# kiliant/zklaim

Hardware: AMD Instinct MI355X
Metric: Groth16 proofs/sec (zklaim gadget, alt_bn128) + G1 MSM GB/s vs HBM roofline (higher is better)
Workload: dtype u32 limbs, Montgomery (254-bit Fq/Fr: 9 x 29-bit in the accumulation, reduction and NTT kernels, 8 x 32-bit elsewhere)

## Files before the change

### zklaim_amd/csrc/msm.hip

```cpp
#include "common.hpp"
#include "fq29.hip.hpp"
#include "host/horner_jac.hpp"
#include "../../include/zkg.h"
#include <algorithm>
#include <chrono>
#include <cstdio>
#include <cstdlib>
#include <cstring>
#include <mutex>

#define ZK_VGPR_CAP(n) __attribute__((amdgpu_num_vgpr((n) / 2)))
static constexpr int ACC29_VGPRS = 192;

namespace zk {

static constexpr int SCALAR_BITS = 255;
template <class F> struct RedGeom { static constexpr int LANES_LOG = sizeof(F) == sizeof(Fq) ? 7 : 6, LANES = 1 << LANES_LOG, THREADS = 4 * LANES; };
static constexpr int RED_L_LOG_TINY = 0, RED_L_LOG_SMALL = 2, RED_L_LOG_LARGE = 4;
static constexpr size_t RED_SMALL_BUCKETS = (size_t)1 << 16, RED_LARGE_BUCKETS = (size_t)1 << 18;
static constexpr int MAX_C = 16;
static constexpr uint32_t HEAVY_S = 512;
static constexpr uint32_t HEAVY_T_MAX = 1024;
static constexpr uint32_t CLASS_HIST_COPIES = 8;
static constexpr int HEAVY_PART_BLOCKS = 512, HEAVY_MERGE_BLOCKS = 128;
// ... 465 lines not shown
    if (cnt > RX_FINE_MAX) { rx_fine_big_bin(tmp, fbits, start, cnt, gb0, cf, of, cur, counts, offsets, sorted, h, heavy_t, class_hist); return; }
    uint32_t ent[RX_FINE_MAX / T];
#pragma unroll
    for (uint32_t j = 0; j < RX_FINE_MAX / T; ++j) {
        uint32_t p = t + j * T;
        ent[j] = p < cnt ? tmp[start + p] : 0xffffffffu;
        if (p < cnt) atomicAdd(&cf[ent[j] >> sh], 1u);
    }
    __syncthreads();
    rx_fine_offsets(cf, of, FB, t, start, gb0, counts, offsets, h, heavy_t, class_hist);
    __syncthreads();
#pragma unroll
    for (uint32_t j = 0; j < RX_FINE_MAX / T; ++j) {
        if (t + j * T >= cnt) continue;
        uint32_t e = ent[j], f = e >> sh;
        bufB[of[f] + atomicAdd(&cur[f], 1u)] = e & low;
    }
    __syncthreads();
    for (uint32_t p = t; p < cnt; p += T) sorted[start + p] = bufB[p];
}

__global__ __launch_bounds__(1024) void k_class_hist(const uint32_t *counts, const uint32_t *offsets, size_t total, uint32_t *class_hist) {
    sort_wave_priority();
    __shared__ uint32_t h[HEAVY_T_MAX + 2];
    const uint32_t heavy_t = heavy_threshold_dev(offsets, total, 1);
    const uint32_t t = threadIdx.x, nc = heavy_t + 2;
    for (uint32_t i = t; i < nc; i += 1024) h[i] = 0;
    __syncthreads();
    size_t gb = (size_t)blockIdx.x * 1024 + t;
    if (gb < total) { uint32_t c = counts[gb]; atomicAdd(&h[c > heavy_t ? heavy_t + 1 : c], 1u); }
    __syncthreads();
    for (uint32_t i = t; i < nc; i += 1024) if (h[i]) atomicAdd(&class_hist[i], h[i]);
}
__global__ __launch_bounds__(1024) void k_order_place(const uint32_t *counts, const uint32_t *offsets, size_t total, const uint32_t *class_hist, uint32_t *class_cursor,
                                                       uint32_t *order, uint32_t *heavy_out) {
    sort_wave_priority();
    __shared__ uint32_t h[HEAVY_T_MAX + 2], first[HEAVY_T_MAX + 2], wave_total[16], threshold;
    const uint32_t t = threadIdx.x, wave = t >> 6, lane = t & 63;
    for (uint32_t i = t; i < HEAVY_T_MAX + 2; i += 1024) h[i] = 0;
    if (t == 0) threshold = heavy_threshold_dev(offsets, total, 1);
    __syncthreads();
    const uint32_t heavy_t = threshold, nc = heavy_t + 2;
    size_t gb = (size_t)blockIdx.x * 1024 + t;
    uint32_t cls = 0, rank = 0;
    if (gb < total) { uint32_t c = counts[gb]; cls = c > heavy_t ? heavy_t + 1 : c; rank = atomicAdd(&h[cls], 1u); }
    uint32_t v0 = 0, v1 = 0, incl = 0;
    if (128 * wave < nc) {
        for (uint32_t k = 0; k < CLASS_HIST_COPIES; ++k) {
            const uint32_t *copy = class_hist + k * (HEAVY_T_MAX + 2);
            if (2 * t < nc) v0 += copy[nc - 1 - 2 * t];
            if (2 * t + 1 < nc) v1 += copy[nc - 2 - 2 * t];
        }
        if (heavy_out && blockIdx.x == 0 && t == 0) *heavy_out = v0;
        incl = v0 + v1;
        for (uint32_t d = 1; d < 64; d <<= 1) { const uint32_t y = __shfl_up(incl, d, 64); if (lane >= d) incl += y; }
    }
    if (lane == 63) wave_total[wave] = incl;
    __syncthreads();
    if (128 * wave < nc) {
        uint32_t before = incl - v0 - v1;
        for (uint32_t k = 0; k < wave; ++k) before += wave_total[k];
        if (2 * t < nc) first[nc - 1 - 2 * t] = before;
        if (2 * t + 1 < nc) first[nc - 2 - 2 * t] = before + v0;
    }
    __syncthreads();
    for (uint32_t i = t; i < nc; i += 1024) if (h[i]) h[i] = first[i] + atomicAdd(&class_cursor[i], h[i]);
    __syncthreads();
    if (gb < total) order[h[cls] + rank] = (uint32_t)gb;
}

template <class F, bool PLAIN>
__global__ __launch_bounds__(256) void k_bucket_accum(const ViewSet<F> views, const uint32_t *sorted, const uint32_t *offsets, const uint32_t *order,
                                                       size_t lanes , XYZZ<F> *buckets, HeavyItem *items,
                                                       HeavyBucket *heavy, uint32_t *counters , SetLayout L) {
    size_t tid = (size_t)blockIdx.x * blockDim.x + threadIdx.x;
    if (tid >= lanes) return;
    const size_t total_buckets = L.buckets;
    const uint32_t set = blockIdx.y;
    const BaseView<F> bases = views.v[set];
    buckets += set * L.buckets; items += set * L.items; heavy += set * L.heavy; counters += 2 * set;
    const uint32_t heavy_t = heavy_threshold_dev(offsets, total_buckets, sizeof(F) > sizeof(Fq) ? 3 : 1);
    const uint32_t gb = order[tid];
    uint32_t k = offsets[gb], end = offsets[gb + 1];
    if (end - k > heavy_t) {
        uint32_t nparts = (end - k + HEAVY_S - 1) / HEAVY_S;
        uint32_t first = atomicAdd(&counters[0], nparts);
        for (uint32_t p = 0; p < nparts; ++p) { uint32_t a = k + p * HEAVY_S; items[first + p] = {a, a + HEAVY_S < end ? a + HEAVY_S : end, gb, nparts == 1}; }
        if (nparts > 1) heavy[atomicAdd(&counters[1], 1u)] = {gb, first, nparts};
        return;
    }
    XYZZ<F> acc = XYZZ<F>::inf();
    if (k < end) {
        uint32_t e = sorted[k], e_next = k + 1 < end ? sorted[k + 1] : 0;
        Affine<F> p = bases.template load<PLAIN>(e, gb);
        while (true) {
            Affine<F> cur = p; uint32_t ce = e;
            ++k;
            if (k < end) { e = e_next; p = bases.template load<PLAIN>(e, gb); if (k + 1 < end) e_next = sorted[k + 1]; }
            if (ce & 1u) cur.y = cur.y.neg();
            acc.madd(cur);
            if (k >= end) break;
        }
    }
    buckets[gb] = acc.normalized();
}

__global__ __launch_bounds__(256) void k_bases_to29(const Affine<Fq> *in, size_t n, Rec64 *out) {
    size_t i = (size_t)blockIdx.x * blockDim.x + threadIdx.x;
    if (i >= n) return;
    const Affine<Fq> a = in[i];
    store_rec64(out + i, f29::to29(a.x), f29::to29(a.y), a.is_inf());
}
ZK_D Affine29 load29(const Rec64 *bases, uint32_t e) { return load_rec64(bases + (e >> 1)); }
ZK_D Rec64 load29_raw(const Rec64 *bases, uint32_t e) { return load_rec64_raw(bases + (e >> 1)); }
template <int WAVES, bool OUT29>
__global__ __launch_bounds__(256, WAVES) ZK_VGPR_CAP(ACC29_VGPRS) void k_bucket_accum29(const Rec64 *bases, size_t level_stride, uint32_t B, const uint32_t *sorted, const uint32_t *offsets, const uint32_t *order,
                                                         size_t lanes, void *buckets_, HeavyItem *items, HeavyBucket *heavy, uint32_t *counters, SetLayout L, int flags ) {
    crit_wave_priority(flags & 2);
    const int resume = flags & 1;
    size_t tid = (size_t)blockIdx.x * blockDim.x + threadIdx.x;
    if (tid >= lanes) return;
    const uint32_t heavy_t = heavy_threshold_dev(offsets, L.buckets, 1);
    const uint32_t gb = order[tid];
    if (level_stride) bases += (size_t)(gb / B) * level_stride;
    uint32_t k = offsets[gb], end = offsets[gb + 1];
    if (end - k > heavy_t) {
        uint32_t nparts = (end - k + HEAVY_S - 1) / HEAVY_S;
        uint32_t first = atomicAdd(&counters[0], nparts);
        const bool single = nparts == 1 && !resume;
        for (uint32_t p = 0; p < nparts; ++p) { uint32_t a = k + p * HEAVY_S; items[first + p] = {a, a + HEAVY_S < end ? a + HEAVY_S : end, gb, single}; }
        if (!single) heavy[atomicAdd(&counters[1], 1u)] = {gb, first, nparts};
        return;
    }
    XYZZ29 acc; bool inf = true;
    acc.x = acc.y = acc.zz = acc.zzz = Fq29::zero();
    if constexpr (OUT29) {
        if (resume) {
            if (k >= end) return;
            const Bucket29 old = load_bucket29_raw(reinterpret_cast<const Bucket29 *>(buckets_) + gb);
            uint32_t any = 0;
#pragma unroll
            for (int j = 0; j < 9; ++j) { acc.x.v[j] = old.x[j]; acc.y.v[j] = old.y[j]; acc.zz.v[j] = old.zz[j]; acc.zzz.v[j] = old.zzz[j]; any |= old.zz[j]; }
            inf = any == 0;
        }
    }
    if (k < end) {
        uint32_t e = sorted[k], e_next = k + 1 < end ? sorted[k + 1] : 0;
        Rec64 p = load29_raw(bases, e);
        while (true) {
            const Rec64 curw = p; const uint32_t ce = e;
            ++k;
            if (k < end) { e = e_next; p = load29_raw(bases, e); if (k + 1 < end) e_next = sorted[k + 1]; }
            const Affine29 cur = unpack_rec64(curw);
            if (!cur.inf) {
                Fq29 bx, by;
#pragma unroll
                for (int j = 0; j < 9; ++j) { bx.v[j] = cur.x[j]; by.v[j] = cur.y[j]; }
                if (ce & 1u) by = f29::neg(f29::S2_1, by);
                if (__builtin_expect(!acc.madd(bx, by, inf), 0)) {
                    XYZZ<Fq> a32 = {f29::from29(acc.x), f29::from29(acc.y), f29::from29(acc.zz), f29::from29(acc.zzz)};
                    a32.madd(Affine<Fq>{f29::from29(bx), f29::from29(f29::norm(by))});
                    if (a32.is_inf()) inf = true;
                    else { acc.x = f29::to29(a32.x.normalized()); acc.y = f29::to29(a32.y.normalized()); acc.zz = f29::to29(a32.zz.normalized()); acc.zzz = f29::to29(a32.zzz.normalized()); }
                }
            }
            if (k >= end) break;
        }
    }
    if constexpr (OUT29) store_bucket29(reinterpret_cast<Bucket29 *>(buckets_) + gb, acc, inf);
    else {
        XYZZ<Fq> *buckets = reinterpret_cast<XYZZ<Fq> *>(buckets_);
        if (inf) buckets[gb] = XYZZ<Fq>::inf().normalized();
        else buckets[gb] = XYZZ<Fq>{f29::from29(acc.x), f29::from29(acc.y), f29::from29(acc.zz), f29::from29(acc.zzz)};
    }
}

template <class F> struct alignas(16) LdsPoint {
    XYZZ<F> p; uint32_t pad[4];
    ZK_D LdsPoint &operator=(const XYZZ<F> &v) { p = v; return *this; }
    ZK_D operator const XYZZ<F> &() const { return p; }
    ZK_D XYZZ<F> normalized() const { return p.normalized(); }
// ... 230 lines not shown
    }
    xyzz29_add_pair(run, cur, r);
    Half29 Q = run;
    for (uint32_t d = 1; d < RED_LANES; d <<= 1) {
        lds_store_half29(sh + t, Q, r);
        __syncthreads();
        if (t + d < RED_LANES) xyzz29_add_pair(Q, lds_load_half29(sh + t + d, r), r);
        __syncthreads();
    }
    const Half29 P = Q;
    lds_store_half29(sh + t, t >= 1 ? Q : Half29::inf(), r); lds_store_half29(sh + RED_LANES + t, T0, r);
    __syncthreads();
    for (uint32_t d = RED_LANES / 2; d >= 1; d >>= 1) {
        if (t < d) { Half29 a = lds_load_half29(sh + t, r); xyzz29_add_pair(a, lds_load_half29(sh + t + d, r), r); lds_store_half29(sh + t, a, r); }
        else if (t >= RED_LANES / 2 && t < RED_LANES / 2 + d) {
            const uint32_t u = RED_LANES + (t - RED_LANES / 2);
            Half29 a = lds_load_half29(sh + u, r); xyzz29_add_pair(a, lds_load_half29(sh + u + d, r), r); lds_store_half29(sh + u, a, r);
        }
        __syncthreads();
    }
    if (t == 0) lds_store_half29(sh + 1, P, r);
    __syncthreads();
    if (threadIdx.x == 0) {
        XYZZ<Fq> E = store_point29(sh[0].p);
        for (int i = 0; i < RED_L_LOG; ++i) E = E.dbl();
        E.add(store_point29(sh[RED_LANES].p));
        out[2 * (size_t)blockIdx.x] = store_point29(sh[1].p); out[2 * (size_t)blockIdx.x + 1] = E.normalized();
    }
}

__global__ __launch_bounds__(2 * RedGeom<Fq>::LANES) void k_bucket_reduce29l(const Bucket29 *buckets, uint32_t B, uint32_t chunks_per_window, XYZZ<Fq> *out,
                                                                             size_t in_set_stride, size_t out_set_stride, int critical) {
    crit_wave_priority(critical);
    constexpr int RED_LANES = RedGeom<Fq>::LANES, NT = 2 * RED_LANES, PER = 8, RED_CHUNK = NT * PER;
    static_assert(RED_CHUNK == (RED_LANES << RED_L_LOG_LARGE), "the lane-form reduction keeps the large reduction's chunks");
    extern __shared__ unsigned char red_smem[];
    LdsPoint29 *sh = reinterpret_cast<LdsPoint29 *>(red_smem);
    const uint32_t i = threadIdx.x;
    const uint32_t w = blockIdx.x / chunks_per_window, ch = blockIdx.x % chunks_per_window;
    const Bucket29 *X = buckets + blockIdx.y * in_set_stride + (size_t)w * B;
    out += blockIdx.y * out_set_stride;
    {
        const uint32_t base = ch * RED_CHUNK + i * PER;
        XYZZ29q run = XYZZ29q::inf(), T0 = XYZZ29q::inf();
        XYZZ29q cur = load_bucket29<true>(X, base + PER - 1, B, 0);
        for (int j = PER - 1; j >= 1; --j) {
            const XYZZ29q nxt = load_bucket29<true>(X, base + j - 1, B, 0);
            xyzz29_add_lane(run, cur);
            xyzz29_add_lane(T0, run);
            cur = nxt;
        }
        xyzz29_add_lane(run, cur);
        sh[i].p = run; sh[NT + i].p = T0;
    }
    __syncthreads();
    const uint32_t t = i >> 1, r = i & 1;
    const Half29 R1 = lds_load_half29(sh + 2 * t + 1, r);
    Half29 Q = lds_load_half29(sh + 2 * t, r);
    xyzz29_add_pair(Q, R1, r);
    Half29 Tp = lds_load_half29(sh + NT + 2 * t, r);
    xyzz29_add_pair(Tp, lds_load_half29(sh + NT + 2 * t + 1, r), r);
    __syncthreads();
    for (uint32_t d = 1; d < RED_LANES; d <<= 1) {
        lds_store_half29(sh + t, Q, r);
        __syncthreads();
        if (t + d < RED_LANES) xyzz29_add_pair(Q, lds_load_half29(sh + t + d, r), r);
        __syncthreads();
    }
    const Half29 P = Q;
    lds_store_half29(sh + t, Q, r);
    __syncthreads();
    Half29 V = t + 1 < RED_LANES ? lds_load_half29(sh + t + 1, r) : Half29::inf();
    xyzz29_add_pair(V, R1, r);
    if (t >= 1) xyzz29_add_pair(V, Q, r);
    __syncthreads();
    lds_store_half29(sh + t, V, r); lds_store_half29(sh + RED_LANES + t, Tp, r);
    __syncthreads();
    for (uint32_t d = RED_LANES / 2; d >= 1; d >>= 1) {
        if (t < d) { Half29 a = lds_load_half29(sh + t, r); xyzz29_add_pair(a, lds_load_half29(sh + t + d, r), r); lds_store_half29(sh + t, a, r); }
        else if (t >= RED_LANES / 2 && t < RED_LANES / 2 + d) {
            const uint32_t u = RED_LANES + (t - RED_LANES / 2);
            Half29 a = lds_load_half29(sh + u, r); xyzz29_add_pair(a, lds_load_half29(sh + u + d, r), r); lds_store_half29(sh + u, a, r);
        }
        __syncthreads();
    }
    if (t == 0) lds_store_half29(sh + 1, P, r);
    __syncthreads();
    if (threadIdx.x < 3) out[3 * (size_t)blockIdx.x + threadIdx.x] = store_point29(threadIdx.x == 0 ? sh[1].p : threadIdx.x == 1 ? sh[RED_LANES].p : sh[0].p);
}


__global__ __launch_bounds__(256) void k_bucket_fold29(const Bucket29 *buckets, const uint32_t *counts, uint32_t W, uint32_t B, Bucket29 *out, int critical) {
    crit_wave_priority(critical);
    const uint32_t b = (blockIdx.x * blockDim.x + threadIdx.x) >> 1, r = threadIdx.x & 1;
    if (b >= B) return;
    Half29 acc = Half29::inf();
    uint32_t w = 0;
    while (w < W && !counts[(size_t)w * B + b]) ++w;
    Half29 cur = w < W ? load_half29<true>(buckets + (size_t)w * B, b, B, r) : Half29::inf();
    while (w < W) {
        uint32_t nw = w + 1;
        while (nw < W && !counts[(size_t)nw * B + b]) ++nw;
        const Half29 nxt = nw < W ? load_half29<true>(buckets + (size_t)nw * B, b, B, r) : Half29::inf();
        xyzz29_add_pair(acc, cur, r);
        cur = nxt; w = nw;
    }
    uint32_t *o = reinterpret_cast<uint32_t *>(out + b) + 9 * r;
#pragma unroll
    for (int i = 0; i < 9; ++i) { o[i] = acc.c0.v[i]; o[18 + i] = acc.c1.v[i]; }
}

static constexpr uint32_t FOLD_THREADS = 256;
template <class F>
__global__ __launch_bounds__(FOLD_THREADS) void k_bucket_fold(const XYZZ<F> *buckets, const uint32_t *counts, uint32_t W, uint32_t B, uint32_t fold_b_log, XYZZ<F> *out, SetLayout L) {
    extern __shared__ unsigned char red_smem[];
    LdsPoint<F> *sh = reinterpret_cast<LdsPoint<F> *>(red_smem);
    const uint32_t t = threadIdx.x, FB = 1u << fold_b_log, slots = FOLD_THREADS >> fold_b_log;
    const uint32_t bl = t & (FB - 1), slot = t >> fold_b_log, b = blockIdx.x * FB + bl;
    buckets += blockIdx.y * L.buckets; out += blockIdx.y * L.folded;
    XYZZ<F> acc = XYZZ<F>::inf();
    if (b < B) for (uint32_t w = slot; w < W; w += slots) if (counts[(size_t)w * B + b]) acc.add(buckets[(size_t)w * B + b]);
// ... 117 lines not shown
    extern __shared__ unsigned char red_smem[];
    LdsPoint<F> *sh = reinterpret_cast<LdsPoint<F> *>(red_smem);
    XYZZ<F> *partials = partials_all + (size_t)blockIdx.y * vec_stride + (size_t)blockIdx.x * (count + 1), *out = partials + count;
    XYZZ<F> acc = XYZZ<F>::inf();
    for (uint32_t i = threadIdx.x; i < count; i += 256) acc.add(partials[i]);
    sh[threadIdx.x] = acc;
    __syncthreads();
    lds_tree_reduce<F>(sh, 256, threadIdx.x, 256, [] { __syncthreads(); });
    if (threadIdx.x == 0) out[0] = sh[0].normalized();
}

struct MsmGroup {
    DevBuf buckets, folded, red_out, heavy_items, heavy_buckets, heavy_partials;
    DevBuf bases29;
    void *host_red = nullptr; size_t host_cap = 0; bool g2 = false, table = false; int nsets = 0;
    int out_index[MSM_MAX_SETS] = {0};
    int red_slots = 2; size_t red_stride = 0;
    uint32_t cpw = 0, red_windows = 0; size_t nred = 0; int chunk_log = 0;
    int host_reserve(size_t bytes) {
        if (bytes <= host_cap) return 0;
        if (host_red) (void)hipHostFree(host_red);
        host_red = nullptr; host_cap = 0;
        if (!hip_ok(hipHostMalloc(&host_red, bytes + 4096, hipHostMallocDefault), "hipHostMalloc", __FILE__, __LINE__)) return 1;
        host_cap = bytes + 4096;
        return 0;
    }
    void release() {
        for (DevBuf *b : {&buckets, &folded, &red_out, &heavy_items, &heavy_buckets, &heavy_partials, &bases29}) b->release();
        if (host_red) (void)hipHostFree(host_red);
        host_red = nullptr; host_cap = 0;
    }
};
struct MsmSortSpace {
    DevBuf digits, hist, counts, offsets, scan_sums, class_hist, order, sorted, rx_tmp, rx_meta, heavy_counters[2];
    void release() { for (DevBuf *b : {&digits, &hist, &counts, &offsets, &scan_sums, &class_hist, &order, &sorted, &rx_tmp, &rx_meta, &heavy_counters[0], &heavy_counters[1]}) b->release(); }
};
struct MsmLaunchMode {
    hipStream_t sort_stream = nullptr;
    uint32_t *heavy_out = nullptr;
    int window = 0;
    bool resume = false;
    bool defer_reduce = false;
    bool heavy_pair = true;
    bool beside = false;
    bool timed = false;
    uint32_t *stream_waits = nullptr;
};
struct MsmJob {
    hipStream_t stream = nullptr; bool own_stream = false;
    MsmSortSpace space;
    MsmGroup group[2];
    MsmGeom g{}; size_t n = 0;
    int window_hint = 0;
    uint32_t merge_hint = 1, merge = 1;
    hipStream_t aux = nullptr; hipEvent_t ev_fork = nullptr, ev_join = nullptr; bool converted_aside = false;
    bool one_pass_sort = false;
    bool critical = false;
    uint32_t w0 = 0, ws = 1;
    bool empty = false;
    bool dev_finish = false;
    uint32_t multi = 1; size_t multi_stride = 0;
    std::mutex mu;
    int ensure_side() {
        if (aux) return ZKG_OK;
        if (hipStreamCreateWithFlags(&aux, hipStreamNonBlocking) == hipSuccess && hipEventCreateWithFlags(&ev_fork, hipEventDisableTiming) == hipSuccess &&
            hipEventCreateWithFlags(&ev_join, hipEventDisableTiming) == hipSuccess) return ZKG_OK;
        release_side(); set_error("msm: side stream"); return ZKG_ERROR;
    }
    void release_side() {
        if (aux) { (void)hipStreamSynchronize(aux); (void)hipStreamDestroy(aux); }
        if (ev_fork) (void)hipEventDestroy(ev_fork);
        if (ev_join) (void)hipEventDestroy(ev_join);
        aux = nullptr; ev_fork = ev_join = nullptr;
    }
    void release_device() {
        space.release();
        for (MsmGroup &gr : group) gr.release();
        release_side();
    }
};
struct MsmLaunchSets { MsmBases by_field[2][MSM_MAX_SETS]; MsmGeom g{}; size_t n = 0; bool empty = false; MsmSortSpace *space = nullptr; };

template <class F>
static int launch_accumulate(MsmJob *job, MsmGroup &gr, const MsmLaunchSets &ls, const uint32_t *d_gather, const MsmLaunchMode &mode, bool time_it) {
    const MsmSortSpace &sp = *ls.space; const MsmBases *sets = ls.by_field[gr.g2 ? 1 : 0];
    const MsmGeom g = ls.g; const size_t n = ls.n, total_buckets = (size_t)g.W * g.B; const unsigned ns = (unsigned)gr.nsets;
    const uint32_t P = job->multi, BP = g.B * P, Wp = g.W / P;
    hipStream_t s = job->stream;
    size_t n_entries_max = n * g.W;
    const size_t max_heavy = std::min(total_buckets, n_entries_max / (sizeof(F) != sizeof(Fq) ? 4 : 8)) + 1,
                 max_items = max_heavy + n_entries_max / HEAVY_S + 1;
    typedef RedGeom<F> RG;
    gr.table = sets[0].level_stride != 0;
    gr.red_windows = gr.table ? P : g.W;
    const size_t red_buckets = (size_t)gr.red_windows * g.B;
    static const char *force_l = getenv("ZKG_RED_L_LOG");
    const int red_l_log = force_l ? atoi(force_l) : red_buckets >= RED_LARGE_BUCKETS ? RED_L_LOG_LARGE : red_buckets > RED_SMALL_BUCKETS ? RED_L_LOG_SMALL : RED_L_LOG_TINY;
    gr.chunk_log = RG::LANES_LOG + red_l_log;
    gr.cpw = (g.B + (1u << gr.chunk_log) - 1) >> gr.chunk_log; gr.nred = (size_t)gr.red_windows * gr.cpw;
    gr.red_slots = 2;
    SetLayout L; L.buckets = total_buckets; L.items = max_items; L.heavy = max_heavy; L.partials = max_items; L.folded = BP; L.red_out = gr.nred * 3;
    if (gr.heavy_items.reserve(ns * max_items * sizeof(HeavyItem)) || gr.heavy_buckets.reserve(ns * max_heavy * sizeof(HeavyBucket)) ||
        gr.heavy_partials.reserve(ns * max_items * sizeof(XYZZ<F>)) ||
        gr.buckets.reserve(ns * total_buckets * std::max(sizeof(XYZZ<F>), sizeof(Bucket29))) || (job->dev_finish && gr.red_out.reserve(ns * L.red_out * sizeof(XYZZ<F>))) || ((gr.red_stride = L.red_out), false) ||
        (gr.table && gr.folded.reserve(ns * (size_t)BP * std::max(sizeof(XYZZ<F>), sizeof(Bucket29)))) || (!job->dev_finish && gr.host_reserve(ns * L.red_out * sizeof(XYZZ<F>)))) return ZKG_ERROR;
    XYZZ<F> *buckets = gr.buckets.as<XYZZ<F>>();
    uint32_t *heavy_counters = sp.heavy_counters[gr.g2 ? 1 : 0].as<uint32_t>();
    ViewSet<F> views;
    for (unsigned i = 0; i < (unsigned)MSM_MAX_SETS; ++i) {
        const MsmBases &b = sets[i < ns ? i : 0];
        views.v[i] = BaseView<F>{reinterpret_cast<const Affine<F> *>(b.p), b.level_stride, d_gather, b.index_sub, BP, b.remap};
    }
    const size_t lanes = gr.table ? std::min(total_buckets, n_entries_max) : total_buckets;
    bool plain = !d_gather;
    for (unsigned i = 0; i < ns; ++i) plain = plain && sets[i].level_stride == 0 && sets[i].index_sub == 0 && !sets[i].remap;
    bool use29 = false; const Rec64 *rec29 = nullptr; size_t stride29 = 0;
    if constexpr (sizeof(F) == sizeof(Fq)) {
        if (ns == 1 && plain) {
            use29 = true;
            if (sets[0].p29) rec29 = reinterpret_cast<const Rec64 *>(sets[0].p29);
            else {
                ZK_HIP(hipStreamWaitEvent(s, job->ev_join, 0));
                if (mode.stream_waits) ++*mode.stream_waits;
                rec29 = gr.bases29.as<Rec64>();
            }
        } else if (ns == 1 && !d_gather && sets[0].p29 && !sets[0].remap && sets[0].index_sub == 0) {
            use29 = true; rec29 = reinterpret_cast<const Rec64 *>(sets[0].p29); stride29 = sets[0].level_stride;
        }
    }
    const bool out29 = use29 && (stride29 == 0 ? !gr.table : (gr.table && ns == 1 && Wp <= 8));
    const int resume = mode.resume ? 1 : 0;
    if (time_it) g_dominant_timer.begin(s);
    if constexpr (sizeof(F) == sizeof(Fq)) {
        static const int waves_env = getenv("ZKG_ACC29_WAVES") ? atoi(getenv("ZKG_ACC29_WAVES")) : 0;
        const int waves29 = waves_env ? waves_env : (mode.beside || gr.table) ? 2 : 3;
        auto launch29 = [&](auto kern) {
            hipLaunchKernelGGL(kern, dim3((unsigned)((lanes + 255) / 256)), dim3(256), 0, s, rec29, stride29, BP, sp.sorted.as<uint32_t>(),
                               sp.offsets.as<uint32_t>(), sp.order.as<uint32_t>(), lanes, (void *)buckets, gr.heavy_items.as<HeavyItem>(),
                               gr.heavy_buckets.as<HeavyBucket>(), heavy_counters, L, resume | (job->critical ? 2 : 0));
        };
        if (use29 && waves29 == 3) { if (out29) launch29(k_bucket_accum29<3, true>); else launch29(k_bucket_accum29<3, false>); }
        else if (use29) { if (out29) launch29(k_bucket_accum29<2, true>); else launch29(k_bucket_accum29<2, false>); }
    }
    auto launch32 = [&](auto kern) {
        hipLaunchKernelGGL(kern, dim3((unsigned)((lanes + 255) / 256), ns), dim3(256), 0, s, views, sp.sorted.as<uint32_t>(), sp.offsets.as<uint32_t>(), sp.order.as<uint32_t>(),
                           lanes, buckets, gr.heavy_items.as<HeavyItem>(), gr.heavy_buckets.as<HeavyBucket>(), heavy_counters, L);
    };
    if (!use29) { if (plain) launch32(k_bucket_accum<F, true>); else launch32(k_bucket_accum<F, false>); }
    if (time_it) g_dominant_timer.end(s);
    if (mode.heavy_pair) {
    hipLaunchKernelGGL(k_heavy_parts<F>, dim3(HEAVY_PART_BLOCKS, ns), dim3(256), 256 * sizeof(LdsPoint<F>), s,
                       views, sp.sorted.as<uint32_t>(), gr.heavy_items.as<HeavyItem>(), heavy_counters, gr.heavy_partials.as<XYZZ<F>>(), buckets, L, (int)out29);
    hipLaunchKernelGGL(k_heavy_merge<F>, dim3(HEAVY_MERGE_BLOCKS, ns), dim3(256), 256 * sizeof(LdsPoint<F>), s,
                       gr.heavy_buckets.as<HeavyBucket>(), heavy_counters, gr.heavy_partials.as<XYZZ<F>>(), buckets, L, (int)out29, resume);
    }
    if (mode.defer_reduce) {
        if (hipGetLastError() != hipSuccess) { set_error("msm kernel launch failed"); return ZKG_ERROR; }
        return ZKG_OK;
    }
    const XYZZ<F> *red_in = buckets; size_t in_stride = L.buckets;
    XYZZ<F> *red_dst = job->dev_finish ? gr.red_out.as<XYZZ<F>>() : reinterpret_cast<XYZZ<F> *>(gr.host_red);
    bool folded29 = false;
    if constexpr (sizeof(F) == sizeof(Fq)) {
        if (gr.table && out29) {
            hipLaunchKernelGGL(k_bucket_fold29, dim3((2 * BP + 255) / 256), dim3(256), 0, s, reinterpret_cast<const Bucket29 *>(buckets), sp.counts.as<uint32_t>(), Wp, BP,
                               gr.folded.as<Bucket29>(), job->critical ? 1 : 0);
            red_in = gr.folded.as<XYZZ<F>>(); in_stride = L.folded; folded29 = true;
        }
    }
    if (gr.table && !folded29) {
        uint32_t slots = 1; while (slots < Wp && slots < 32) slots <<= 1;
        uint32_t fold_b_log = 0; while ((FOLD_THREADS >> (fold_b_log + 1)) >= slots) ++fold_b_log;
// ... 133 lines not shown
    if (t == 0) store_norm_dev<F>(out + POINT_WORDS<F> * ((size_t)w * gridDim.y + set), sh[0]);
}
template <class F> static void launch_combine(dim3 grid, hipStream_t s, const XYZZ<F> *red, uint32_t cpw, int slots, int chunk_log, size_t set_stride, uint32_t *out) {
    hipLaunchKernelGGL((k_msm_combine<F, COMBINE_THREADS<F>>), grid, dim3(COMBINE_THREADS<F>), combine_lds_bytes<F>(cpw), s, red, cpw, slots, chunk_log, set_stride, out);
}
template <class F> __global__ __launch_bounds__(64) void k_msm_store_inf(uint32_t *out, uint32_t count) {
    const uint32_t i = blockIdx.x * blockDim.x + threadIdx.x;
    if (i < count) store_norm_dev(out + POINT_WORDS<F> * (size_t)i, XYZZ<F>::inf());
}
template <class F> __global__ __launch_bounds__(256) void k_jac_to_records(const uint32_t *jac, size_t count, XYZZ<F> *rec) {
    const size_t i = (size_t)blockIdx.x * blockDim.x + threadIdx.x;
    if (i >= count) return;
    const uint32_t *in = jac + POINT_WORDS<F> * i;
    F X, Y, Z;
    load_limbs(X, in); load_limbs(Y, in + sizeof(F) / 4); load_limbs(Z, in + 2 * (sizeof(F) / 4));
    rec[i] = Z.is_zero() ? XYZZ<F>::inf() : XYZZ<F>{X, Y, F::one(), F::one()};
}

static int sort_digits(MsmJob *job, MsmLaunchSets &ls, const uint32_t *d_scalars, bool mont, const uint32_t *d_gather, const MsmLaunchMode &mode) {
    MsmSortSpace &sp = *ls.space;
    const MsmGeom g0 = job->g; const size_t n0 = job->n;
    if (job->merge > 1) { job->g.W /= job->merge; job->g.Wt = job->g.W; job->n *= job->merge; }
    if (job->multi > 1) { job->g.W *= job->multi; job->g.Wt = job->g.W; }
    const MsmGeom g = ls.g = job->g; const size_t n = ls.n = job->n;
    hipStream_t s = mode.sort_stream ? mode.sort_stream : job->stream;
    const size_t total = (size_t)g.W * g.B;
    uint32_t slice_len = (uint32_t)std::min<size_t>(65536, std::max<size_t>(4096, ((n + 15) / 16 + 1023) / 1024 * 1024));
    uint32_t S = (uint32_t)std::max<size_t>(1, (n + slice_len - 1) / slice_len);
    size_t nblk = (total + 1024 * SCAN_ITEMS - 1) / (1024 * SCAN_ITEMS);
    if (nblk > 1024) { set_error("msm: too many buckets for the block scan"); return ZKG_ERROR; }
    if (sp.digits.reserve(std::max<size_t>(1, n * g.W) * 4) || sp.hist.reserve((size_t)g.W * S * g.B * 4) || sp.counts.reserve(total * 4) ||
        sp.offsets.reserve((total + 1) * 4) || sp.scan_sums.reserve(1024 * 4) || sp.class_hist.reserve((CLASS_HIST_COPIES + 1) * (HEAVY_T_MAX + 2) * 4) ||
        sp.order.reserve(total * 4) || sp.sorted.reserve(std::max<size_t>(1, n * g.W) * 4)) return ZKG_ERROR;
    uint32_t *digits = sp.digits.as<uint32_t>(), *hist = sp.hist.as<uint32_t>(), *counts = sp.counts.as<uint32_t>(),
             *offsets = sp.offsets.as<uint32_t>(), *sums = sp.scan_sums.as<uint32_t>(), *chist = sp.class_hist.as<uint32_t>();
    uint32_t cbits = 6;
    static const uint32_t bin_avg = getenv("ZKG_RX_AVG") ? (uint32_t)atoi(getenv("ZKG_RX_AVG")) : RX_BIN_AVG;
    while (cbits < RX_MAX_CBITS && cbits + 1 < g.c - 1 && (n >> cbits) > bin_avg) ++cbits;
    const bool two_pass = !job->one_pass_sort && g.c >= 12 && n >= 49152 && (n >> cbits) <= RX_FINE_MAX && n <= ((size_t)1 << (31 - (g.c - 1 - cbits)));
    {
        ZeroList zl{};
        int k = 0;
        zl.p[k] = chist; zl.words[k++] = (CLASS_HIST_COPIES + 1) * (HEAVY_T_MAX + 2);
        for (int f = 0; f < 2; ++f) if (job->group[f].nsets) {
            if (sp.heavy_counters[f].reserve(8 * MSM_MAX_SETS)) return ZKG_ERROR;
            zl.p[k] = sp.heavy_counters[f].as<uint32_t>(); zl.words[k++] = 2 * MSM_MAX_SETS;
        }
        if (two_pass) {
            const uint32_t nbins = g.W << cbits;
            if (sp.rx_meta.reserve((2 * (size_t)nbins + g.W) * 4)) return ZKG_ERROR;
            zl.p[k] = sp.rx_meta.as<uint32_t>(); zl.words[k++] = 2 * nbins + g.W;
        }
        const dim3 dg((unsigned)((n0 + 255) / 256));
        const bool four = !d_gather && (n0 & 3) == 0 && g0.w0 == 0 && g0.ws == 1 && g0.W == g0.Wt;
        const dim3 dg4((unsigned)((n0 / 4 + 255) / 256));
        if (job->multi > 1) {
            const dim3 dgm(dg.x, job->multi);
            if (g0.c == 16) hipLaunchKernelGGL(k_digits_multi<16>, dgm, dim3(256), 0, s, d_scalars, job->multi_stride, n0, (int)mont, job->merge, digits, zl);
            else if (g0.c == 12) hipLaunchKernelGGL(k_digits_multi<12>, dgm, dim3(256), 0, s, d_scalars, job->multi_stride, n0, (int)mont, job->merge, digits, zl);
            else hipLaunchKernelGGL(k_digits_multi_any, dgm, dim3(256), 0, s, d_scalars, job->multi_stride, n0, (int)mont, g0, job->merge, digits, zl);
        }
        else if (four && g0.c == 16) hipLaunchKernelGGL(k_digits_c4<16>, dg4, dim3(256), 0, s, d_scalars, n0, (int)mont, g0, digits, zl);
        else if (four && g0.c == 12) hipLaunchKernelGGL(k_digits_c4<12>, dg4, dim3(256), 0, s, d_scalars, n0, (int)mont, g0, digits, zl);
        else if (g0.c == 16) hipLaunchKernelGGL(k_digits_c<16>, dg, dim3(256), 0, s, d_scalars, d_gather, n0, (int)mont, g0, digits, zl);
        else if (g0.c == 12) hipLaunchKernelGGL(k_digits_c<12>, dg, dim3(256), 0, s, d_scalars, d_gather, n0, (int)mont, g0, digits, zl);
        else hipLaunchKernelGGL(k_digits, dg, dim3(256), 0, s, d_scalars, d_gather, n0, (int)mont, g0, digits, zl);
    }
    if (two_pass) {
        const uint32_t fbits = g.c - 1 - cbits, CB = 1u << cbits, nbins = g.W * CB, S1 = (uint32_t)((n + RX_SLICE - 1) / RX_SLICE);
        if (sp.rx_tmp.reserve(n * g.W * 4)) return ZKG_ERROR;
        uint32_t *cnt = sp.rx_meta.as<uint32_t>(), *cursor = cnt + nbins, *wtot = cursor + nbins, *tmp = sp.rx_tmp.as<uint32_t>();
        const size_t fine_lds = (RX_FINE_MAX + 3 * (1u << fbits)) * 4;
        hipLaunchKernelGGL(k_rx_count, dim3(S1, g.W), dim3(1024), 0, s, digits, n, fbits, cbits, cnt, wtot);
        static const int wg_env = getenv("ZKG_SORT_WG") ? atoi(getenv("ZKG_SORT_WG")) : 0;
        const bool half = (wg_env ? wg_env == 512 : mode.sort_stream != nullptr) && fbits <= 9;
        if (half) {
            const uint32_t S2 = (uint32_t)((n + 512 * RX_PER_THREAD - 1) / (512 * RX_PER_THREAD));
            hipLaunchKernelGGL(k_rx_scatter<512>, dim3(S2, g.W), dim3(512), (512 * RX_PER_THREAD + 4 * RX_MAX_CB + 8) * 4, s, digits, n, fbits, cbits, cnt, wtot, g.W, cursor, tmp, offsets + total);
            hipLaunchKernelGGL(k_rx_fine<512>, dim3(CB, g.W), dim3(512), fine_lds, s, tmp, fbits, cbits, g.B, cnt, wtot, counts, offsets, total, chist,
                               sp.sorted.as<uint32_t>());
        } else {
            hipLaunchKernelGGL(k_rx_scatter<1024>, dim3(S1, g.W), dim3(1024), (RX_SLICE + 4 * RX_MAX_CB + 8) * 4, s, digits, n, fbits, cbits, cnt, wtot, g.W, cursor, tmp, offsets + total);
            hipLaunchKernelGGL(k_rx_fine<1024>, dim3(CB, g.W), dim3(1024), fine_lds, s, tmp, fbits, cbits, g.B, cnt, wtot, counts, offsets, total, chist,
                               sp.sorted.as<uint32_t>());
        }
    } else {
    hipLaunchKernelGGL(k_hist, dim3(S, g.W), dim3(SORT_THREADS), g.B * 4, s, digits, n, g.B, S, slice_len, hist);
    hipLaunchKernelGGL(k_colscan, dim3((unsigned)((total + 255) / 256)), dim3(256), 0, s, hist, g.B, S, total, counts);
    hipLaunchKernelGGL(k_scan_blocks, dim3((unsigned)nblk), dim3(1024), 0, s, counts, offsets, sums, total);
    hipLaunchKernelGGL(k_scan_sums, dim3(1), dim3(1024), 0, s, sums, (uint32_t)nblk, offsets + total);
    hipLaunchKernelGGL(k_scan_apply, dim3((unsigned)nblk), dim3(1024), 0, s, offsets, sums, total);
    hipLaunchKernelGGL(k_place, dim3(S, g.W), dim3(SORT_THREADS), g.B * 4, s, digits, n, g.B, S, slice_len, hist, offsets, sp.sorted.as<uint32_t>());
    hipLaunchKernelGGL(k_class_hist, dim3((unsigned)((total + 1023) / 1024)), dim3(1024), 0, s, counts, offsets, total, chist);
    }
    hipLaunchKernelGGL(k_order_place, dim3((unsigned)((total + 1023) / 1024)), dim3(1024), 0, s, counts, offsets, total, chist, chist + CLASS_HIST_COPIES * (HEAVY_T_MAX + 2), sp.order.as<uint32_t>(), mode.heavy_out);
    if (hipGetLastError() != hipSuccess) { set_error("msm sort launch failed"); return ZKG_ERROR; }
    return ZKG_OK;
}

MsmJob *msm_job_create(hipStream_t s, bool own_stream, bool high_priority) {
    MsmJob *j = new MsmJob();
    j->stream = s;
    if (own_stream) {
        int prio_lo = 0, prio_hi = 0;
        (void)hipDeviceGetStreamPriorityRange(&prio_lo, &prio_hi);
        if (!hip_ok(hipStreamCreateWithPriority(&j->stream, hipStreamNonBlocking, high_priority ? prio_hi : prio_lo), "hipStreamCreate", __FILE__, __LINE__)) { delete j; return nullptr; }
        j->own_stream = true;
    }
    return j;
}
void msm_job_set_window(MsmJob *j, int c) { if (j) j->window_hint = c; }
bool crit_priority_enabled() { static const bool on = !(getenv("ZKG_CRIT_PRIO") && atoi(getenv("ZKG_CRIT_PRIO")) == 0); return on; }
void msm_job_set_critical(MsmJob *j, bool critical) { if (j) j->critical = critical && crit_priority_enabled(); }
void msm_job_set_row_merge(MsmJob *j, uint32_t f) { if (j) j->merge_hint = f ? f : 1; }
void msm_job_set_skewed(MsmJob *j, bool skewed) { if (j) j->one_pass_sort = skewed; }
void msm_job_set_window_subset(MsmJob *j, uint32_t w0, uint32_t ws) { if (j) { j->w0 = w0; j->ws = ws ? ws : 1; } }
hipStream_t msm_job_stream(MsmJob *j) { return j->stream; }
void msm_job_destroy(MsmJob *j) {
    if (!j) return;
    j->release_device();
    if (j->own_stream) (void)hipStreamDestroy(j->stream);
    delete j;
}

static MsmJob g_default_job;
struct HostScalarsStats { uint32_t pieces = 0, waits = 0, heavy[8] = {0}, pair[8] = {0}; };
struct PieceStep {
    DevBuf scalars; MsmSortSpace space;
// ... 507 lines not shown
```

Measured before the change: 56.44.

## Restructure large bucket reduction tail to quad-lane point adds with fewer barriers

```diff
diff --git a/zklaim_amd/csrc/msm.hip b/zklaim_amd/csrc/msm.hip
--- a/zklaim_amd/csrc/msm.hip
+++ b/zklaim_amd/csrc/msm.hip
@@ -932,7 +932,7 @@
 __global__ __launch_bounds__(2 * RedGeom<Fq>::LANES) void k_bucket_reduce29l(const Bucket29 *buckets, uint32_t B, uint32_t chunks_per_window, XYZZ<Fq> *out,
                                                                              size_t in_set_stride, size_t out_set_stride, int critical) {
     crit_wave_priority(critical);
-    constexpr int RED_LANES = RedGeom<Fq>::LANES, NT = 2 * RED_LANES, PER = 8, RED_CHUNK = NT * PER;
+    constexpr int RED_LANES = RedGeom<Fq>::LANES, NT = 2 * RED_LANES, NQ = NT / 4, PER = 8, RED_CHUNK = NT * PER;
     static_assert(RED_CHUNK == (RED_LANES << RED_L_LOG_LARGE), "the lane-form reduction keeps the large reduction's chunks");
     extern __shared__ unsigned char red_smem[];
     LdsPoint29 *sh = reinterpret_cast<LdsPoint29 *>(red_smem);
@@ -951,42 +951,55 @@
             cur = nxt;
         }
         xyzz29_add_lane(run, cur);
-        sh[i].p = run; sh[NT + i].p = T0;
-    }
-    __syncthreads();
-    const uint32_t t = i >> 1, r = i & 1;
-    const Half29 R1 = lds_load_half29(sh + 2 * t + 1, r);
-    Half29 Q = lds_load_half29(sh + 2 * t, r);
-    xyzz29_add_pair(Q, R1, r);
-    Half29 Tp = lds_load_half29(sh + NT + 2 * t, r);
-    xyzz29_add_pair(Tp, lds_load_half29(sh + NT + 2 * t + 1, r), r);
-    __syncthreads();
-    for (uint32_t d = 1; d < RED_LANES; d <<= 1) {
-        lds_store_half29(sh + t, Q, r);
-        __syncthreads();
-        if (t + d < RED_LANES) xyzz29_add_pair(Q, lds_load_half29(sh + t + d, r), r);
-        __syncthreads();
-    }
-    const Half29 P = Q;
-    lds_store_half29(sh + t, Q, r);
-    __syncthreads();
-    Half29 V = t + 1 < RED_LANES ? lds_load_half29(sh + t + 1, r) : Half29::inf();
-    xyzz29_add_pair(V, R1, r);
-    if (t >= 1) xyzz29_add_pair(V, Q, r);
-    __syncthreads();
-    lds_store_half29(sh + t, V, r); lds_store_half29(sh + RED_LANES + t, Tp, r);
-    __syncthreads();
-    for (uint32_t d = RED_LANES / 2; d >= 1; d >>= 1) {
-        if (t < d) { Half29 a = lds_load_half29(sh + t, r); xyzz29_add_pair(a, lds_load_half29(sh + t + d, r), r); lds_store_half29(sh + t, a, r); }
-        else if (t >= RED_LANES / 2 && t < RED_LANES / 2 + d) {
-            const uint32_t u = RED_LANES + (t - RED_LANES / 2);
-            Half29 a = lds_load_half29(sh + u, r); xyzz29_add_pair(a, lds_load_half29(sh + u + d, r), r); lds_store_half29(sh + u, a, r);
-        }
-        __syncthreads();
-    }
-    if (t == 0) lds_store_half29(sh + 1, P, r);
-    __syncthreads();
-    if (threadIdx.x < 3) out[3 * (size_t)blockIdx.x + threadIdx.x] = store_point29(threadIdx.x == 0 ? sh[1].p : threadIdx.x == 1 ? sh[RED_LANES].p : sh[0].p);
+        const uint32_t at = (i & 3) * NQ + (i >> 2);
+        sh[at].p = run; sh[NT + at].p = T0;
+    }
+    __syncthreads();
+    const uint32_t t = i >> 2, q = i & 3;
+    LdsPoint29 *const hi = sh + NT;
+    XYZZ29q Q, acc;
+#pragma unroll 1
+    for (uint32_t k = 0; k < 2; ++k) {
+        const LdsPoint29 *e = sh + k * NT + t;
+        XYZZ29q a = e[3 * NQ].p;
+#pragma unroll 1
+        for (int j = 2; j >= 0; --j) xyzz29_add_quad(a, e[j * NQ].p, q);
+        if (k == 0) Q = a; else acc = a;
+    }
+    int step = 0;
+#pragma unroll 1
+    for (uint32_t d = 1; d < NQ; d <<= 1, ++step) {
+        LdsPoint29 *buf = step & 1 ? hi : sh;
+        if (q == 0) buf[t].p = Q;
+        __syncthreads();
+        if (t + d < NQ) xyzz29_add_quad(Q, buf[t + d].p, q);
+    }
+    if (q == 0) sh[t].p = Q;
+    if (i == 0) hi[2 * NQ].p = Q;
+    __syncthreads();
+    XYZZ29q S = t + 1 < NQ ? sh[t + 1].p : XYZZ29q::inf();
+    XYZZ29q V = XYZZ29q::inf();
+#pragma unroll 1
+    for (int j = 3; j >= 1; --j) {
+        xyzz29_add_quad(S, sh[j * NQ + t].p, q);
+        xyzz29_add_quad(V, S, q);
+    }
+    if (t >= 1) xyzz29_add_quad(V, Q, q);
+    if (q == 0) { hi[t].p = V; hi[NQ + t].p = acc; }
+    __syncthreads();
+#pragma unroll 1
+    for (uint32_t d = NQ / 2; d >= 1; d >>= 1) {
+        const bool second = t >= NQ / 2;
+        const uint32_t u = second ? NQ + (t - NQ / 2) : t;
+        if ((second ? t - NQ / 2 : t) < d) { XYZZ29q a = hi[u].p; xyzz29_add_quad(a, hi[u + d].p, q); if (q == 0) hi[u].p = a; }
+        __syncthreads();
+    }
+    if (t < 3) {
+        const XYZZ29q r = hi[t == 0 ? 2 * NQ : t == 1 ? NQ : 0].p;
+        Fq v = f29::from29(quad_select29(q, r.x, r.y, r.zz, r.zzz));
+        if (r.is_inf()) v = q == 1 ? Fq::one().normalized() : Fq::zero();
+        reinterpret_cast<Fq *>(out + 3 * (size_t)blockIdx.x + t)[q] = v;
+    }
 }
 
 
```

After: 56.81, median of 2. About the same (+0.7%).

## Precompute per-lane bucket plan in order placement for 29-bit accumulation

Applied to the files above, without the earlier changes.

```diff
diff --git a/zklaim_amd/csrc/msm.hip b/zklaim_amd/csrc/msm.hip
--- a/zklaim_amd/csrc/msm.hip
+++ b/zklaim_amd/csrc/msm.hip
@@ -521,8 +521,9 @@
     __syncthreads();
     for (uint32_t i = t; i < nc; i += 1024) if (h[i]) atomicAdd(&class_hist[i], h[i]);
 }
+constexpr uint32_t PLAN_HEAVY = 0x80000000u;
 __global__ __launch_bounds__(1024) void k_order_place(const uint32_t *counts, const uint32_t *offsets, size_t total, const uint32_t *class_hist, uint32_t *class_cursor,
-                                                       uint32_t *order, uint32_t *heavy_out) {
+                                                       uint32_t *order, uint32_t *heavy_out, const uint32_t *sorted, uint4 *plan) {
     sort_wave_priority();
     __shared__ uint32_t h[HEAVY_T_MAX + 2], first[HEAVY_T_MAX + 2], wave_total[16], threshold;
     const uint32_t t = threadIdx.x, wave = t >> 6, lane = t & 63;
@@ -531,8 +532,11 @@
     __syncthreads();
     const uint32_t heavy_t = threshold, nc = heavy_t + 2;
     size_t gb = (size_t)blockIdx.x * 1024 + t;
-    uint32_t cls = 0, rank = 0;
-    if (gb < total) { uint32_t c = counts[gb]; cls = c > heavy_t ? heavy_t + 1 : c; rank = atomicAdd(&h[cls], 1u); }
+    uint32_t cls = 0, rank = 0, c = 0, begin = 0, head = 0;
+    if (gb < total) {
+        c = counts[gb]; cls = c > heavy_t ? heavy_t + 1 : c; rank = atomicAdd(&h[cls], 1u);
+        if (plan) { begin = offsets[gb]; if (c) head = sorted[begin]; }
+    }
     uint32_t v0 = 0, v1 = 0, incl = 0;
     if (128 * wave < nc) {
         for (uint32_t k = 0; k < CLASS_HIST_COPIES; ++k) {
@@ -555,7 +559,11 @@
     __syncthreads();
     for (uint32_t i = t; i < nc; i += 1024) if (h[i]) h[i] = first[i] + atomicAdd(&class_cursor[i], h[i]);
     __syncthreads();
-    if (gb < total) order[h[cls] + rank] = (uint32_t)gb;
+    if (gb < total) {
+        const uint32_t pos = h[cls] + rank;
+        order[pos] = (uint32_t)gb;
+        if (plan) plan[pos] = make_uint4((uint32_t)gb | (c > heavy_t ? PLAN_HEAVY : 0u), begin, begin + c, head);
+    }
 }
 
 template <class F, bool PLAIN>
@@ -603,17 +611,17 @@
 ZK_D Affine29 load29(const Rec64 *bases, uint32_t e) { return load_rec64(bases + (e >> 1)); }
 ZK_D Rec64 load29_raw(const Rec64 *bases, uint32_t e) { return load_rec64_raw(bases + (e >> 1)); }
 template <int WAVES, bool OUT29>
-__global__ __launch_bounds__(256, WAVES) ZK_VGPR_CAP(ACC29_VGPRS) void k_bucket_accum29(const Rec64 *bases, size_t level_stride, uint32_t B, const uint32_t *sorted, const uint32_t *offsets, const uint32_t *order,
-                                                         size_t lanes, void *buckets_, HeavyItem *items, HeavyBucket *heavy, uint32_t *counters, SetLayout L, int flags ) {
+__global__ __launch_bounds__(256, WAVES) ZK_VGPR_CAP(ACC29_VGPRS) void k_bucket_accum29(const Rec64 *bases, size_t level_stride, uint32_t B, const uint32_t *sorted, const uint4 *plan,
+                                                         size_t lanes, void *buckets_, HeavyItem *items, HeavyBucket *heavy, uint32_t *counters, int flags ) {
     crit_wave_priority(flags & 2);
     const int resume = flags & 1;
     size_t tid = (size_t)blockIdx.x * blockDim.x + threadIdx.x;
     if (tid >= lanes) return;
-    const uint32_t heavy_t = heavy_threshold_dev(offsets, L.buckets, 1);
-    const uint32_t gb = order[tid];
+    const uint4 pl = plan[tid];
+    const uint32_t gb = pl.x & ~PLAN_HEAVY;
     if (level_stride) bases += (size_t)(gb / B) * level_stride;
-    uint32_t k = offsets[gb], end = offsets[gb + 1];
-    if (end - k > heavy_t) {
+    uint32_t k = pl.y; const uint32_t end = pl.z;
+    if (pl.x & PLAN_HEAVY) {
         uint32_t nparts = (end - k + HEAVY_S - 1) / HEAVY_S;
         uint32_t first = atomicAdd(&counters[0], nparts);
         const bool single = nparts == 1 && !resume;
@@ -623,6 +631,11 @@
     }
     XYZZ29 acc; bool inf = true;
     acc.x = acc.y = acc.zz = acc.zzz = Fq29::zero();
+    uint32_t e = pl.w, e_next = 0; Rec64 p;
+    if (k < end) {
+        p = load29_raw(bases, e);
+        if (k + 1 < end) e_next = sorted[k + 1];
+    }
     if constexpr (OUT29) {
         if (resume) {
             if (k >= end) return;
@@ -634,8 +647,6 @@
         }
     }
     if (k < end) {
-        uint32_t e = sorted[k], e_next = k + 1 < end ? sorted[k + 1] : 0;
-        Rec64 p = load29_raw(bases, e);
         while (true) {
             const Rec64 curw = p; const uint32_t ce = e;
             ++k;
@@ -1170,8 +1181,9 @@
     }
 };
 struct MsmSortSpace {
-    DevBuf digits, hist, counts, offsets, scan_sums, class_hist, order, sorted, rx_tmp, rx_meta, heavy_counters[2];
-    void release() { for (DevBuf *b : {&digits, &hist, &counts, &offsets, &scan_sums, &class_hist, &order, &sorted, &rx_tmp, &rx_meta, &heavy_counters[0], &heavy_counters[1]}) b->release(); }
+    DevBuf digits, hist, counts, offsets, scan_sums, class_hist, order, plan, sorted, rx_tmp, rx_meta, heavy_counters[2];
+    bool planned = false;
+    void release() { for (DevBuf *b : {&digits, &hist, &counts, &offsets, &scan_sums, &class_hist, &order, &plan, &sorted, &rx_tmp, &rx_meta, &heavy_counters[0], &heavy_counters[1]}) b->release(); }
 };
 struct MsmLaunchMode {
     hipStream_t sort_stream = nullptr;
@@ -1218,6 +1230,10 @@
     }
 };
 struct MsmLaunchSets { MsmBases by_field[2][MSM_MAX_SETS]; MsmGeom g{}; size_t n = 0; bool empty = false; MsmSortSpace *space = nullptr; };
+static bool launch_takes_accum29(const MsmJob *job, const MsmLaunchSets &ls, const uint32_t *d_gather) {
+    const MsmBases &b = ls.by_field[0][0];
+    return job->group[0].nsets == 1 && !d_gather && b.index_sub == 0 && !b.remap && (b.level_stride == 0 || b.p29);
+}
 
 template <class F>
 static int launch_accumulate(MsmJob *job, MsmGroup &gr, const MsmLaunchSets &ls, const uint32_t *d_gather, const MsmLaunchMode &mode, bool time_it) {
@@ -1254,17 +1270,16 @@
     for (unsigned i = 0; i < ns; ++i) plain = plain && sets[i].level_stride == 0 && sets[i].index_sub == 0 && !sets[i].remap;
     bool use29 = false; const Rec64 *rec29 = nullptr; size_t stride29 = 0;
     if constexpr (sizeof(F) == sizeof(Fq)) {
-        if (ns == 1 && plain) {
-            use29 = true;
+        use29 = launch_takes_accum29(job, ls, d_gather);
+        if (use29 && !sp.planned) { set_error("msm: the sort wrote no lane plan for a 29-bit accumulation"); return ZKG_ERROR; }
+        if (use29 && plain) {
             if (sets[0].p29) rec29 = reinterpret_cast<const Rec64 *>(sets[0].p29);
             else {
                 ZK_HIP(hipStreamWaitEvent(s, job->ev_join, 0));
                 if (mode.stream_waits) ++*mode.stream_waits;
                 rec29 = gr.bases29.as<Rec64>();
             }
-        } else if (ns == 1 && !d_gather && sets[0].p29 && !sets[0].remap && sets[0].index_sub == 0) {
-            use29 = true; rec29 = reinterpret_cast<const Rec64 *>(sets[0].p29); stride29 = sets[0].level_stride;
-        }
+        } else if (use29) { rec29 = reinterpret_cast<const Rec64 *>(sets[0].p29); stride29 = sets[0].level_stride; }
     }
     const bool out29 = use29 && (stride29 == 0 ? !gr.table : (gr.table && ns == 1 && Wp <= 8));
     const int resume = mode.resume ? 1 : 0;
@@ -1274,8 +1289,8 @@
         const int waves29 = waves_env ? waves_env : (mode.beside || gr.table) ? 2 : 3;
         auto launch29 = [&](auto kern) {
             hipLaunchKernelGGL(kern, dim3((unsigned)((lanes + 255) / 256)), dim3(256), 0, s, rec29, stride29, BP, sp.sorted.as<uint32_t>(),
-                               sp.offsets.as<uint32_t>(), sp.order.as<uint32_t>(), lanes, (void *)buckets, gr.heavy_items.as<HeavyItem>(),
-                               gr.heavy_buckets.as<HeavyBucket>(), heavy_counters, L, resume | (job->critical ? 2 : 0));
+                               sp.plan.as<uint4>(), lanes, (void *)buckets, gr.heavy_items.as<HeavyItem>(),
+                               gr.heavy_buckets.as<HeavyBucket>(), heavy_counters, resume | (job->critical ? 2 : 0));
         };
         if (use29 && waves29 == 3) { if (out29) launch29(k_bucket_accum29<3, true>); else launch29(k_bucket_accum29<3, false>); }
         else if (use29) { if (out29) launch29(k_bucket_accum29<2, true>); else launch29(k_bucket_accum29<2, false>); }
@@ -1475,6 +1490,8 @@
     if (sp.digits.reserve(std::max<size_t>(1, n * g.W) * 4) || sp.hist.reserve((size_t)g.W * S * g.B * 4) || sp.counts.reserve(total * 4) ||
         sp.offsets.reserve((total + 1) * 4) || sp.scan_sums.reserve(1024 * 4) || sp.class_hist.reserve((CLASS_HIST_COPIES + 1) * (HEAVY_T_MAX + 2) * 4) ||
         sp.order.reserve(total * 4) || sp.sorted.reserve(std::max<size_t>(1, n * g.W) * 4)) return ZKG_ERROR;
+    sp.planned = launch_takes_accum29(job, ls, d_gather);
+    if (sp.planned && sp.plan.reserve(total * sizeof(uint4))) return ZKG_ERROR;
     uint32_t *digits = sp.digits.as<uint32_t>(), *hist = sp.hist.as<uint32_t>(), *counts = sp.counts.as<uint32_t>(),
              *offsets = sp.offsets.as<uint32_t>(), *sums = sp.scan_sums.as<uint32_t>(), *chist = sp.class_hist.as<uint32_t>();
     uint32_t cbits = 6;
@@ -1536,7 +1553,8 @@
     hipLaunchKernelGGL(k_place, dim3(S, g.W), dim3(SORT_THREADS), g.B * 4, s, digits, n, g.B, S, slice_len, hist, offsets, sp.sorted.as<uint32_t>());
     hipLaunchKernelGGL(k_class_hist, dim3((unsigned)((total + 1023) / 1024)), dim3(1024), 0, s, counts, offsets, total, chist);
     }
-    hipLaunchKernelGGL(k_order_place, dim3((unsigned)((total + 1023) / 1024)), dim3(1024), 0, s, counts, offsets, total, chist, chist + CLASS_HIST_COPIES * (HEAVY_T_MAX + 2), sp.order.as<uint32_t>(), mode.heavy_out);
+    hipLaunchKernelGGL(k_order_place, dim3((unsigned)((total + 1023) / 1024)), dim3(1024), 0, s, counts, offsets, total, chist, chist + CLASS_HIST_COPIES * (HEAVY_T_MAX + 2), sp.order.as<uint32_t>(), mode.heavy_out,
+                       sp.sorted.as<uint32_t>(), sp.planned ? sp.plan.as<uint4>() : (uint4 *)nullptr);
     if (hipGetLastError() != hipSuccess) { set_error("msm sort launch failed"); return ZKG_ERROR; }
     return ZKG_OK;
 }
```

Result: no change. 58.65 before, 58.82 after, median of 3 (+0.3%).
